# LasseWolter/laughter-detection-icsi

Hardware: AMD Instinct MI355X
Metric: 1 s@16 kHz segments/sec (featurize+ResNet fwd/bwd) (higher is better)
Workload: dtype f32 (64->64 and 32->32 convolutions: f16x2 split operands with per-tile power-of-two scales, f32 accumulate; error vs float64 within 1.5x of the exact-f32 kernels'); 1 GPU; BASELINE configs[2]: end-to-end featurize (HIP fbank 44 mel) + ResNetBigger resnet_base fwd/bwd + clip + Adam, random labels, dropout 0.5; global_batch=512, parallelism=dp1, overlap_wgrad=False, overlap_wgrad_small=True, bf16x3_convs=True, f16x2_convs=True, relu_bits=True, virtual_a1=True

## Files before the change

include/lad_hip.h:

```cpp
#ifndef LAD_HIP_H
#define LAD_HIP_H

#include <stdint.h>

#ifdef __cplusplus
extern "C" {
#endif

#define LAD_VERSION 100

enum lad_status {
    LAD_OK = 0,
    LAD_ERR_INVALID = -1,
    LAD_ERR_HIP = -2,
    LAD_ERR_NOMEM = -3,
    LAD_NOT_COVERED = 1
};

int lad_version(void);
const char *lad_last_error(void);

enum lad_pad_mode {
    LAD_PAD_KALDI_MIRROR = 0,
    LAD_PAD_CENTER_REFLECT = 1,
// ... 159 lines not shown
int lad_stem_bwd_onepass(const float *feat, const float *weight, const float *dy, const float *coef, const float *gamma,
                         const double *moments, float *workspace, float *dw, float *dgamma, float *dbeta, int64_t batch, int32_t H,
                         int32_t W, int32_t cout, void *stream);
int64_t lad_stem_wgrad_workspace_floats(void);
int lad_stem_wgrad(const float *feat, const float *dout, float *workspace, float *dw, int64_t batch, int32_t H,
                   int32_t W, int32_t cout, void *stream);
int lad_stem_wgrad_bn(const float *feat, const float *dy, const float *x, const float *weight, const float *coef,
                      const float *bcoef, float *workspace, float *dw, int64_t batch, int32_t H, int32_t W, int32_t cout,
                      void *stream);
int64_t lad_stem_bn_bwd_groups(int64_t batch, int32_t H, int32_t W);
int lad_stem_bn_bwd_sums(const float *feat, const float *weight, const float *dy, const float *coef, float *partials,
                         int64_t batch, int32_t H, int32_t W, int32_t cout, void *stream);

int lad_bn_finalize(float *stat_partials, int64_t n_tiles, int32_t channels, int64_t count, const float *gamma,
                    const float *beta, float *running_mean, float *running_var, float momentum, float *coef,
                    void *stream);
int lad_bn_finalize_pair(float *stat_partials_a, float *stat_partials_b, int64_t n_tiles, int32_t channels, int64_t count,
                         const float *gamma_a, const float *beta_a, float *running_mean_a, float *running_var_a, float *coef_a,
                         const float *gamma_b, const float *beta_b, float *running_mean_b, float *running_var_b, float *coef_b,
                         float momentum, void *stream);
int lad_bn_act(const float *x, const float *coef, const float *res, const float *res_coef, float *y, int64_t batch,
               int32_t H, int32_t W, int32_t channels, int32_t relu, void *stream);
int64_t lad_bn_bwd_workspace_floats(int32_t channels);
int lad_bn_bwd(const float *dy, const float *y, const float *x, const float *coef, const float *gamma,
               const float *xs, const float *scoef, const float *sgamma, float *dx, float *aux, float *dgamma,
               float *dbeta, float *dsgamma, float *dsbeta, float *workspace, float *bcoef, float *pre_partials,
               int64_t pre_tiles, int64_t batch, int32_t H, int32_t W, int32_t channels, int32_t relu, int32_t mode,
               void *stream);
int lad_bn_act_bits(const float *x, const float *coef, const float *res, const float *res_coef, float *y,
                    uint64_t *y_bits, int64_t batch, int32_t H, int32_t W, int32_t channels, void *stream);
int lad_bn_bwd_bits(const float *dy, const uint64_t *y_bits, const float *x, const float *coef, const float *gamma,
                    float *dx, float *dgamma, float *dbeta, float *workspace, float *bcoef, float *pre_partials,
                    int64_t pre_tiles, int64_t batch, int32_t H, int32_t W, int32_t channels, void *stream);
int lad_conv_fwd_bnstat(const float *in, const float *wt, const float *addend, float *out, float *stat_partials,
                        const float *bn_x, const float *bn_y, const float *bn_coef, int64_t batch, int32_t H, int32_t W,
                        int32_t cin, int32_t cout, int32_t taps, void *stream);

int lad_pool_fwd(const float *x, float *pooled, int64_t batch, int32_t H, int32_t W, int32_t channels, void *stream);
int lad_pool_bwd(const float *dpooled, float *dx, int64_t batch, int32_t H, int32_t W, int32_t channels, void *stream);
int64_t lad_head_workspace_floats(int64_t batch, int32_t F);
int lad_head_fwd_train(const float *const *params, const float *pooled, int64_t batch, int32_t F, const float *drop1,
                       const float *drop2, const int32_t *labels, float momentum, float *h, float *stats,
                       float *probs, float *metrics, void *stream);
int lad_head_fwd_train_rng(const float *const *params, const float *pooled, int64_t batch, int32_t F, float *drop1, float *drop2, float keep,
                           uint64_t seed, int64_t *rng_counter, int64_t *nbt, int32_t n_nbt, const int32_t *labels, float momentum,
                           float *h, float *stats, float *probs, float *metrics, void *stream);
int lad_head_fwd_eval(const float *const *params, const float *pooled, int64_t batch, int32_t F, float *probs,
                      void *stream);
int lad_bce_metrics(const float *probs, const int32_t *labels, int64_t n, float *metrics, void *stream);
int lad_head_bwd(const float *const *params, float *const *grads, const float *pooled, const float *h,
                 const float *stats, const float *probs, const float *dprobs, int64_t batch, int32_t F,
                 const float *drop1, const float *drop2, const int32_t *labels, float *workspace, float *dpooled,
                 void *stream);

int64_t lad_f16_packed_weight_halfs(int32_t cout, int32_t cin, int32_t taps);
int lad_f16_pack_weights(const float *w, int32_t cout, int32_t cin, int32_t taps, void *wt, void *stream);
int lad_f16_stem_fwd(const float *feat, const float *weight, const float *scale, const float *shift, void *out,
                     int64_t batch, int32_t H, int32_t W, int32_t cout, int64_t frame_stride, int64_t frames_avail,
                     void *stream);
int lad_f16_conv_fwd(const void *in, const void *wt, const float *scale, const float *shift, const void *addend, void *out,
                     int64_t batch, int32_t H, int32_t W, int32_t cin, int32_t cout, int32_t taps, int32_t relu,
                     void *stream);
int lad_f16_conv_s2_fwd(const void *in, const void *wt, const float *scale, const float *shift, void *out, int64_t batch,
                        int32_t H, int32_t W, int32_t cin, int32_t cout, int32_t taps, int32_t relu, void *stream);
int lad_f16_block_fwd(const void *x, const void *wt1, const float *scale1, const float *shift1, const void *wt2,
                      const float *scale2, const float *shift2, void *y, int64_t batch, int32_t H, int32_t W, int32_t channels,
                      void *stream);
int lad_f16_block_fwd_stem_rows(const void *stream_act, int64_t stream_rows, int64_t stream_row0, const float *feat, int64_t frames_avail,
                                const float *stem_weight, const float *stem_scale, const float *stem_shift, const void *wt1,
                                const float *scale1, const float *shift1, const void *wt2, const float *scale2, const float *shift2, void *y,
                                int64_t batch, int32_t H, int32_t W, void *stream);
int lad_f16_conv_s2_strips_fwd(const void *act, const void *wt, const float *scale, const float *shift, void *out, const void *wt_sc,
                               const float *scale_sc, const float *shift_sc, void *out_sc, int64_t n_windows, int32_t H, int32_t W,
                               int32_t band, int32_t strip_rows, int64_t bottom_image0, int64_t stream_row0, int64_t act_rows,
                               int32_t out_rows, void *stream);
int lad_f16_tail_fwd(const void *act, int64_t n_windows, int32_t H, int32_t W, int32_t band, int32_t strip_rows, int64_t bot_img0,
                     int64_t stream_row0, int32_t phases, int64_t phase_img, int64_t act_rows, const void *const *conv_params,
                     const float *const *head_params, int32_t F, float *probs, void *stream);
int lad_f16_conv_s2_fwd_windows(const void *act, const void *wt, const float *scale, const float *shift, void *out,
                                int64_t n_windows, int32_t H, int32_t W, int32_t band, int32_t cin, int32_t cout, int32_t taps,
                                int32_t relu, void *stream);
int lad_f16_conv_s2_fwd_mapped(const void *act, const void *wt, const float *scale, const float *shift, void *out,
                               int64_t n_windows, int32_t H, int32_t W, int32_t band, int32_t strip_rows, int64_t bottom_image0,
                               int64_t stream_row0, int32_t phases, int64_t phase_rows, int64_t act_rows, int32_t out_rows,
                               int32_t cin, int32_t cout, int32_t taps, int32_t relu, void *stream);
int lad_f16_conv_s2_fwd_sc(const void *in, const void *wt, const float *scale, const float *shift, void *out, const void *wt_sc,
                           const float *scale_sc, const float *shift_sc, void *out_sc, int64_t batch, int32_t H, int32_t W,
                           int32_t cin, int32_t cout, int32_t relu, void *stream);
int lad_f16_conv_s2_fwd_mapped_sc(const void *act, const void *wt, const float *scale, const float *shift, void *out,
                                  const void *wt_sc, const float *scale_sc, const float *shift_sc, void *out_sc, int64_t n_windows,
                                  int32_t H, int32_t W, int32_t band, int32_t strip_rows, int64_t bottom_image0, int64_t stream_row0,
                                  int32_t phases, int64_t phase_rows, int64_t act_rows, int32_t out_rows, int32_t cin, int32_t cout,
                                  int32_t relu, void *stream);
int lad_f16_pool_fwd(const void *x, float *pooled, int64_t batch, int32_t H, int32_t W, int32_t channels, void *stream);

int32_t lad_grad_sumsq_partials(void);
int lad_grad_sumsq(const float *grad, int64_t n, float *partials, int64_t *step_counter, void *stream);
int lad_grad_accumulate(float *acc, const float *grad, int64_t n, double scale, void *stream);
int lad_adam_step(float *param, float *grad, float *exp_avg, float *exp_avg_sq, int64_t n,
                  const float *sumsq_partials, double grad_scale, double max_norm, double lr, double beta1,
                  double beta2, double eps, int64_t step, const int64_t *step_counter, int32_t zero_grad,
                  float *norm_out, void *stream);

enum lad_runs_dtype { LAD_RUNS_F32 = 0, LAD_RUNS_F64 = 1 };
int32_t lad_runs_tile_frames(void);
int32_t lad_runs_max_thresholds(void);
// ... 107 lines not shown
```

laughter-detection-icsi_amd/_hip.py:

```python
import ctypes
import os

import numpy as np
import torch

_HERE = os.path.dirname(os.path.abspath(__file__))
LIB_PATH = os.environ.get("LAD_HIP_LIB") or os.path.join(_HERE, "liblad_hip.so")

c_void_p = ctypes.c_void_p
c_int = ctypes.c_int
c_i64 = ctypes.c_int64
c_float = ctypes.c_float
c_double = ctypes.c_double
c_i32 = ctypes.c_int32
c_float_p = ctypes.POINTER(ctypes.c_float)


class LadHipError(RuntimeError):
    pass


class FbankCfg(ctypes.Structure):
    _fields_ = [("n_fft", ctypes.c_int32), ("frame_len", ctypes.c_int32), ("hop", ctypes.c_int32),
                ("n_mels", ctypes.c_int32), ("n_mfcc", ctypes.c_int32), ("pad_mode", ctypes.c_int32),
# ... 56 lines not shown
    "lad_conv_fwd_eval": (c_int, [c_void_p] * 6 + [c_i64, c_i32, c_i32, c_i32, c_i32, c_i32, c_i32, c_void_p]),
    "lad_conv_s2_fwd_eval": (c_int, [c_void_p] * 5 + [c_i64, c_i32, c_i32, c_i32, c_i32, c_i32, c_i32, c_void_p]),
    "lad_upsample2": (c_int, [c_void_p, c_void_p, c_i64, c_i32, c_i32, c_i32, c_void_p]),
    "lad_conv_s2_dgrad": (c_int, [c_void_p] * 3 + [c_i64, c_i32, c_i32, c_i32, c_i32, c_i32, c_i32, c_void_p]),
    "lad_conv_s2_wgrad_workspace_floats": (c_i64, [c_i32, c_i32, c_i32]),
    "lad_conv_s2_fwd_fused": (c_int, [c_void_p] * 8 + [c_i64, c_i32, c_i32, c_i32, c_i32, c_void_p]),
    "lad_conv_s2_dgrad_partials": (c_i64, [c_i64, c_i32, c_i32]),
    "lad_conv_s2b3_packed_weight_bytes": (c_i64, []),
    "lad_conv_s2b3_pack_weights": (c_int, [c_void_p, c_void_p, c_void_p, c_void_p]),
    "lad_conv_s2b3_fwd": (c_int, [c_void_p] * 7 + [c_i64, c_i32, c_i32, c_void_p]),
    "lad_conv_s2b3_dgrad_packed_weight_bytes": (c_i64, []),
    "lad_conv_s2b3_dgrad_pack_weights": (c_int, [c_void_p, c_void_p, c_void_p, c_void_p]),
    "lad_conv_s2b3_pack_weights_pair": (c_int, [c_void_p] * 5),
    "lad_conv_s2b3_dgrad_partials": (c_i64, [c_i64, c_i32, c_i32]),
    "lad_conv_s2b3_dgrad": (c_int, [c_void_p] * 8 + [c_i64, c_i32, c_i32, c_void_p]),
    "lad_conv_s2_dgrad_fused_bnstat": (c_int, [c_void_p] * 9 + [c_i64, c_i32, c_i32, c_i32, c_i32, c_void_p]),
    "lad_conv_s2_dgrad_fused": (c_int, [c_void_p] * 5 + [c_i64, c_i32, c_i32, c_i32, c_i32, c_void_p]),
    "lad_conv_s2_wgrad_fused_workspace_floats": (c_i64, [c_i32, c_i32]),
    "lad_conv_s2_wgrad_fused": (c_int, [c_void_p] * 7 + [c_i64, c_i32, c_i32, c_i32, c_i32, c_void_p]),
    "lad_conv_s2_wgrad": (c_int, [c_void_p] * 5 + [c_i64, c_i32, c_i32, c_i32, c_i32, c_i32, c_void_p]),
    "lad_conv_wgrad_workspace_floats": (c_i64, [c_i32, c_i32, c_i32]),
    "lad_conv_wgrad": (c_int, [c_void_p] * 5 + [c_i64, c_i32, c_i32, c_i32, c_i32, c_i32, c_void_p]),
    "lad_stem_fwd": (c_int, [c_void_p] * 4 + [c_i64, c_i32, c_i32, c_i32, c_void_p]),
    "lad_stem_fwd_eval": (c_int, [c_void_p] * 5 + [c_i64, c_i32, c_i32, c_i32, c_i64, c_i64, c_void_p]),
    "lad_stem_wgrad_workspace_floats": (c_i64, []),
    "lad_stem_wgrad": (c_int, [c_void_p] * 4 + [c_i64, c_i32, c_i32, c_i32, c_void_p]),
    "lad_stem_wgrad_bn": (c_int, [c_void_p] * 8 + [c_i64, c_i32, c_i32, c_i32, c_void_p]),
    "lad_stem_bn_bwd_groups": (c_i64, [c_i64, c_i32, c_i32]),
    "lad_stem_bn_bwd_sums": (c_int, [c_void_p] * 5 + [c_i64, c_i32, c_i32, c_i32, c_void_p]),
    "lad_bn_finalize": (c_int, [c_void_p, c_i64, c_i32, c_i64, c_void_p, c_void_p, c_void_p, c_void_p, c_float,
                                c_void_p, c_void_p]),
    "lad_stem_moments_workspace_doubles": (c_i64, []),
    "lad_stem_moments_doubles": (c_i64, []),
    "lad_stem_bn_stats": (c_int, [c_void_p] * 6 + [c_float] + [c_void_p] * 3 + [c_i64, c_i32, c_i32, c_i32, c_void_p]),
    "lad_stem_bwd_onepass_workspace_floats": (c_i64, []),
    "lad_stem_bwd_onepass": (c_int, [c_void_p] * 10 + [c_i64, c_i32, c_i32, c_i32, c_void_p]),
    "lad_bn_finalize_pair": (c_int, [c_void_p, c_void_p, c_i64, c_i32, c_i64] + [c_void_p] * 10 + [c_float, c_void_p]),
    "lad_bn_act": (c_int, [c_void_p] * 5 + [c_i64, c_i32, c_i32, c_i32, c_i32, c_void_p]),
    "lad_bn_bwd_workspace_floats": (c_i64, [c_i32]),
    "lad_bn_act_bits": (c_int, [c_void_p] * 6 + [c_i64, c_i32, c_i32, c_i32, c_void_p]),
    "lad_bn_bwd_bits": (c_int, [c_void_p] * 11 + [c_i64, c_i64, c_i32, c_i32, c_i32, c_void_p]),
    "lad_bn_bwd": (c_int, [c_void_p] * 17 + [c_i64, c_i64, c_i32, c_i32, c_i32, c_i32, c_i32, c_void_p]),
    "lad_conv_fwd_bnstat": (c_int, [c_void_p] * 8 + [c_i64, c_i32, c_i32, c_i32, c_i32, c_i32, c_void_p]),
    "lad_pool_fwd": (c_int, [c_void_p, c_void_p, c_i64, c_i32, c_i32, c_i32, c_void_p]),
    "lad_pool_bwd": (c_int, [c_void_p, c_void_p, c_i64, c_i32, c_i32, c_i32, c_void_p]),
    "lad_head_workspace_floats": (c_i64, [c_i64, c_i32]),
    "lad_head_fwd_train": (c_int, [c_void_p, c_void_p, c_i64, c_i32, c_void_p, c_void_p, c_void_p, c_float,
                                   c_void_p, c_void_p, c_void_p, c_void_p, c_void_p]),
    "lad_head_fwd_train_rng": (c_int, [c_void_p, c_void_p, c_i64, c_i32, c_void_p, c_void_p, c_float, ctypes.c_uint64, c_void_p, c_void_p, c_i32,
                                       c_void_p, c_float, c_void_p, c_void_p, c_void_p, c_void_p, c_void_p]),
    "lad_head_fwd_eval": (c_int, [c_void_p, c_void_p, c_i64, c_i32, c_void_p, c_void_p]),
    "lad_bce_metrics": (c_int, [c_void_p, c_void_p, c_i64, c_void_p, c_void_p]),
    "lad_head_bwd": (c_int, [c_void_p] * 7 + [c_i64, c_i32] + [c_void_p] * 6),
    "lad_f16_packed_weight_halfs": (c_i64, [c_i32, c_i32, c_i32]),
    "lad_f16_pack_weights": (c_int, [c_void_p, c_i32, c_i32, c_i32, c_void_p, c_void_p]),
    "lad_f16_stem_fwd": (c_int, [c_void_p] * 5 + [c_i64, c_i32, c_i32, c_i32, c_i64, c_i64, c_void_p]),
    "lad_f16_conv_fwd": (c_int, [c_void_p] * 6 + [c_i64, c_i32, c_i32, c_i32, c_i32, c_i32, c_i32, c_void_p]),
    "lad_f16_block_fwd": (c_int, [c_void_p] * 8 + [c_i64, c_i32, c_i32, c_i32, c_void_p]),
    "lad_f16_conv_s2_fwd_sc": (c_int, [c_void_p] * 9 + [c_i64, c_i32, c_i32, c_i32, c_i32, c_i32, c_void_p]),
    "lad_f16_conv_s2_fwd_mapped_sc": (c_int, [c_void_p] * 9 + [c_i64, c_i32, c_i32, c_i32, c_i32, c_i64, c_i64, c_i32, c_i64, c_i64, c_i32,
                                              c_i32, c_i32, c_i32, c_void_p]),
    "lad_f16_conv_s2_fwd": (c_int, [c_void_p] * 5 + [c_i64, c_i32, c_i32, c_i32, c_i32, c_i32, c_i32, c_void_p]),
    "lad_f16_conv_s2_fwd_windows": (c_int, [c_void_p] * 5 + [c_i64, c_i32, c_i32, c_i32, c_i32, c_i32, c_i32, c_i32, c_void_p]),
    "lad_f16_conv_s2_fwd_mapped": (c_int, [c_void_p] * 5 + [c_i64, c_i32, c_i32, c_i32, c_i32, c_i64, c_i64, c_i32, c_i64, c_i64, c_i32,
                                                          c_i32, c_i32, c_i32, c_i32, c_void_p]),
    "lad_f16_block_fwd_stem_rows": (c_int, [c_void_p, c_i64, c_i64, c_void_p, c_i64] + [c_void_p] * 10 + [c_i64, c_i32, c_i32, c_void_p]),
    "lad_f16_conv_s2_strips_fwd": (c_int, [c_void_p] * 9 + [c_i64, c_i32, c_i32, c_i32, c_i32, c_i64, c_i64, c_i64, c_i32, c_void_p]),
    "lad_f16_tail_fwd": (c_int, [c_void_p, c_i64, c_i32, c_i32, c_i32, c_i32, c_i64, c_i64, c_i32, c_i64, c_i64, c_void_p, c_void_p, c_i32,
                                 c_void_p, c_void_p]),
    "lad_f16_pool_fwd": (c_int, [c_void_p, c_void_p, c_i64, c_i32, c_i32, c_i32, c_void_p]),
    "lad_grad_sumsq_partials": (c_i32, []),
    "lad_grad_sumsq": (c_int, [c_void_p, c_i64, c_void_p, c_void_p, c_void_p]),
    "lad_grad_accumulate": (c_int, [c_void_p, c_void_p, c_i64, c_double, c_void_p]),
    "lad_adam_step": (c_int, [c_void_p] * 4 + [c_i64, c_void_p] + [c_double] * 6 + [c_i64, c_void_p, c_i32, c_void_p, c_void_p]),
    "lad_runs_tile_frames": (c_i32, []),
    "lad_runs_max_thresholds": (c_i32, []),
    "lad_runs_workspace_bytes": (c_i64, [c_i64, c_i64, c_i32]),
    "lad_runs_count": (c_int, [c_void_p, c_i32, c_i64, c_i64, ctypes.POINTER(c_double), c_i32, c_void_p, c_void_p]),
    "lad_runs_fill": (c_int, [c_void_p, c_i32, c_i64, c_i64, ctypes.POINTER(c_double), c_i32, c_void_p,
                              ctypes.POINTER(c_i32), c_void_p, c_i64, c_void_p]),
    "lad_score_max_min_lengths": (c_i32, []),
    "lad_score_workspace_bytes": (c_i64, [c_i64, c_i64, c_i32, c_i32]),
    "lad_score_runs": (c_int, [c_void_p, c_void_p, ctypes.POINTER(c_i32), c_i64, c_i64, c_i32, c_void_p, c_void_p,
                               ctypes.POINTER(c_i32), ctypes.POINTER(c_i32), c_i64, c_void_p, ctypes.POINTER(c_double),
                               ctypes.POINTER(c_double), c_i32, c_void_p, c_void_p, c_void_p]),
    "lad_score_events_workspace_bytes": (c_i64, [c_i64, c_i64, c_i32, c_i32, c_i64]),
    "lad_score_events": (c_int, [c_void_p, c_void_p, ctypes.POINTER(c_i32), c_i64, c_i64, c_i32, c_void_p, c_void_p,
                                 ctypes.POINTER(c_i32), ctypes.POINTER(c_i32), c_i64, c_void_p, ctypes.POINTER(c_double),
                                 ctypes.POINTER(c_double), c_i32, c_i32, c_i32, c_void_p, c_void_p, c_void_p]),
    "lad_binarize_max_settings": (c_i32, []),
    "lad_binarize_workspace_bytes": (c_i64, [c_i64, c_i64, c_i32]),
    "lad_binarize_count": (c_int, [c_void_p, c_i32, c_i64, c_i64, ctypes.POINTER(c_double), ctypes.POINTER(c_double), c_i32,
                                   c_void_p, c_void_p]),
    "lad_binarize_fill": (c_int, [c_void_p, c_i32, c_i64, c_i64] + [ctypes.POINTER(c_double)] * 3
                          + [c_i32, c_void_p, ctypes.POINTER(c_double), c_void_p, ctypes.POINTER(c_i32), c_void_p, c_void_p, c_i64,
                             c_void_p]),
    "lad_viterbi_max_settings": (c_i32, []),
    "lad_viterbi_table_entries": (c_i32, []),
    "lad_viterbi_workspace_bytes": (c_i64, [c_i64, c_i64, c_i32]),
    "lad_viterbi_count": (c_int, [c_void_p, c_i32, c_i64, c_i64, c_void_p] + [ctypes.POINTER(c_i32)] * 3
                          + [c_i32, c_void_p, c_void_p, c_void_p]),
    "lad_viterbi_fill": (c_int, [c_void_p, ctypes.POINTER(c_i32), c_i64, c_i64, c_i32, c_void_p, c_i64, c_void_p]),
    "lad_surface_max_levels": (c_i32, []),
    "lad_surface_tile_frames": (c_i32, []),
    "lad_surface_workspace_bytes": (c_i64, [c_i64, c_i64, c_i64, c_i32, c_i32]),
    "lad_score_surface": (c_int, [c_void_p, c_i32, c_i64, c_i64, ctypes.POINTER(c_double), c_i32, c_void_p, c_void_p,
# ... 116 lines not shown
```

laughter-detection-icsi_amd/csrc/head.hip:

```cpp
#include "lad_common.h"
#include "lad_device.h"
#include "lad_philox.h"

namespace {
using namespace lad;

#ifdef LAD_STAMP
__device__ unsigned long long lad_dbg_head[64];
#define LAD_HEAD_STAMP(k) if (threadIdx.x == 0) lad_dbg_head[k] = __builtin_amdgcn_s_memtime();
#else
#define LAD_HEAD_STAMP(k)
#endif

constexpr float BN_EPS = 1e-5f;
constexpr int HID = 32;
constexpr int HEAD_THREADS = 1024;
constexpr int MAX_F = 128;
constexpr int CH = 64;

struct HeadArgs {
    int B, F;
    const float *g2, *b2;
    float *rm2, *rv2;
    const float *W1, *bias1;
// ... 524 lines not shown
        if (worker) {
            for (int b = g; b < nb; b += KS) {
                const float4 dv = *reinterpret_cast<const float4 *>(dh_s + b * DHS + tj * TJ);
                const float dd[TJ] = {dv.x, dv.y, dv.z, dv.w};
                float zz[TF];
#pragma unroll
                for (int y = 0; y < TF; ++y) zz[y] = z_s[b * (MAX_F + 1) + min(tf * TF + y, MAX_F - 1)];
#pragma unroll
                for (int x = 0; x < TJ; ++x)
#pragma unroll
                    for (int y = 0; y < TF; ++y) wacc[x][y] = fmaf(dd[x], zz[y], wacc[x][y]);
            }
        }
        __syncthreads();
    }
    {
        float *part = z_s;
        if (worker) {
#pragma unroll
            for (int x = 0; x < TJ; ++x)
#pragma unroll
                for (int y = 0; y < TF; ++y) {
                    const int f = tf * TF + y;
                    if (f < F) part[(g * HID + tj * TJ + x) * F + f] = wacc[x][y];
                }
        }
        __syncthreads();
        for (int idx = tid; idx < HID * F; idx += nt) {
            float sacc = part[idx];
            for (int q = 1; q < KS; ++q) sacc += part[q * HID * F + idx];
            gr_out.dW1[idx] = sacc;
        }
        __syncthreads();
    }
    LAD_HEAD_STAMP(22)
    col_dot2(dh, nullptr, nullptr, nullptr, B, HID, gr_out.dbias1, nullptr, scratch);
    LAD_HEAD_STAMP(23)
    col_dot2(dz, pooled, mean2, istd2, B, F, ca, cb, scratch);
    __syncthreads();
    for (int f = tid; f < F; f += nt) {
        gr_out.db2[f] = ca[f];
        gr_out.dg2[f] = cb[f];
    }
    LAD_HEAD_STAMP(24)
    batched<12, F2>(tid, B * F, nt, [&](int idx) { return F2{pooled[idx], dz[idx]}; },
                   [&](int idx, const F2 &v) {
                       const int f = idx % F;
                       const float xh = (v.a - mu2[f]) * is2[f];
                       dpooled[idx] = kk2[f] * (v.b - ca[f] / (float)B - xh * cb[f] / (float)B);
                   });
    LAD_HEAD_STAMP(25)
}

int check_head(const HeadArgs &a) {
    using namespace lad;
    LAD_REQUIRE(a.B >= 1 && a.F >= 1 && a.F <= MAX_F, "head: F must be 1..%d (got %d), B >= 1", MAX_F, a.F);
    LAD_REQUIRE(a.g2 && a.b2 && a.rm2 && a.rv2 && a.W1 && a.bias1 && a.g3 && a.b3 && a.rm3 && a.rv3 && a.W2 && a.bias2,
                "head: null parameter pointer");
    return LAD_OK;
}

}

extern "C" int lad_pool_fwd(const float *x, float *pooled, int64_t batch, int32_t H, int32_t W, int32_t channels, void *stream) {
    using namespace lad;
    LAD_REQUIRE(x && pooled, "lad_pool_fwd: null buffer");
    LAD_REQUIRE(H >= 4 && W >= 4 && channels >= 1, "lad_pool_fwd: AvgPool2d(4) needs H, W >= 4");
    if (batch == 0) return LAD_OK;
    const int PH = H / 4, PW = W / 4;
    const int64_t n = batch * channels * PH * PW;
    hipLaunchKernelGGL(pool_fwd_kernel, dim3((unsigned)ceil_div(n, 256)), dim3(256), 0, (hipStream_t)stream, x, pooled, batch, H + 1,
                       W + 1, channels, PH, PW);
    return check_launch("pool_fwd_kernel");
}

extern "C" int lad_pool_bwd(const float *dpooled, float *dx, int64_t batch, int32_t H, int32_t W, int32_t channels, void *stream) {
    using namespace lad;
    LAD_REQUIRE(dpooled && dx, "lad_pool_bwd: null buffer");
    LAD_REQUIRE(H >= 4 && W >= 4 && channels >= 1, "lad_pool_bwd: AvgPool2d(4) needs H, W >= 4");
    if (batch == 0) return LAD_OK;
    const int64_t n = batch * (H + 1) * (W + 1) * channels;
    hipLaunchKernelGGL(pool_bwd_kernel, dim3((unsigned)std::min<int64_t>(ceil_div(n, 256), 4096)), dim3(256), 0, (hipStream_t)stream,
                       dpooled, dx, batch, H + 1, W + 1, channels, H / 4, W / 4);
    return check_launch("pool_bwd_kernel");
}

static HeadArgs make_args(const float *const *p, int64_t B, int32_t F, const float *m1, const float *m2, const int32_t *labels,
                          float momentum) {
    HeadArgs a;
    a.B = (int)B; a.F = F;
    a.g2 = p[0]; a.b2 = p[1]; a.rm2 = (float *)p[2]; a.rv2 = (float *)p[3];
    a.W1 = p[4]; a.bias1 = p[5];
    a.g3 = p[6]; a.b3 = p[7]; a.rm3 = (float *)p[8]; a.rv3 = (float *)p[9];
    a.W2 = p[10]; a.bias2 = p[11];
    a.m1 = m1; a.m2 = m2; a.labels = (const int *)labels; a.momentum = momentum;
    a.keep = 1.f; a.seed = 0; a.rng_counter = nullptr; a.nbt = nullptr; a.n_nbt = 0;
    return a;
}

extern "C" int64_t lad_head_workspace_floats(int64_t batch, int32_t F) { return batch * (3 * HID + F); }

extern "C" int lad_head_fwd_train(const float *const *params, const float *pooled, int64_t batch, int32_t F, const float *drop1,
                                  const float *drop2, const int32_t *labels, float momentum, float *h, float *stats, float *probs,
                                  float *metrics, void *stream) {
    using namespace lad;
    LAD_REQUIRE(params && pooled && h && stats && probs && metrics, "lad_head_fwd_train: null buffer");
    LAD_REQUIRE(batch < (1 << 24), "lad_head_fwd_train: batch too large for the single-workgroup train head");
    HeadArgs a = make_args(params, batch, F, drop1, drop2, labels, momentum);
    int rc = check_head(a);
    if (rc) return rc;
    hipLaunchKernelGGL(head_fwd_train_kernel, dim3(1), dim3(HEAD_THREADS), 0, (hipStream_t)stream, a, pooled, h, stats, probs, metrics);
    return check_launch("head_fwd_train_kernel");
}

extern "C" int lad_head_fwd_train_rng(const float *const *params, const float *pooled, int64_t batch, int32_t F, float *drop1, float *drop2,
                                      float keep, uint64_t seed, int64_t *rng_counter, int64_t *nbt, int32_t n_nbt, const int32_t *labels,
                                      float momentum, float *h, float *stats, float *probs, float *metrics, void *stream) {
    using namespace lad;
    LAD_REQUIRE(params && pooled && h && stats && probs && metrics, "lad_head_fwd_train_rng: null buffer");
    LAD_REQUIRE(batch >= 2, "lad_head_fwd_train_rng: batch statistics need at least two samples");
    const bool drop = keep < 1.0f;
    LAD_REQUIRE(!drop || (keep > 0.f && drop1 && drop2 && rng_counter && F % 4 == 0), "lad_head_fwd_train_rng: dropout needs mask buffers, a counter and F %% 4 == 0");
    LAD_REQUIRE(n_nbt >= 0 && n_nbt <= HEAD_THREADS - 64 && (n_nbt == 0 || nbt), "lad_head_fwd_train_rng: bad counter list");
    HeadArgs a = make_args(params, batch, F, drop ? drop1 : nullptr, drop ? drop2 : nullptr, labels, momentum);
    int rc = check_head(a);
    if (rc) return rc;
    a.keep = keep; a.seed = seed; a.rng_counter = drop ? (long long *)rng_counter : nullptr; a.nbt = (long long *)nbt; a.n_nbt = n_nbt;
    hipLaunchKernelGGL(head_fwd_train_kernel, dim3(1), dim3(HEAD_THREADS), 0, (hipStream_t)stream, a, pooled, h, stats, probs, metrics);
    return check_launch("head_fwd_train_kernel");
}

extern "C" int lad_head_fwd_eval(const float *const *params, const float *pooled, int64_t batch, int32_t F, float *probs, void *stream) {
    using namespace lad;
    LAD_REQUIRE(params && pooled && probs, "lad_head_fwd_eval: null buffer");
    if (batch == 0) return LAD_OK;
    HeadArgs a = make_args(params, batch, F, nullptr, nullptr, nullptr, 0.f);
    int rc = check_head(a);
    if (rc) return rc;
    hipLaunchKernelGGL(head_fwd_eval_kernel, dim3((unsigned)ceil_div(batch, 256)), dim3(256), 0, (hipStream_t)stream, a, pooled, probs);
    return check_launch("head_fwd_eval_kernel");
}

extern "C" int lad_bce_metrics(const float *probs, const int32_t *labels, int64_t n, float *metrics, void *stream) {
    using namespace lad;
    LAD_REQUIRE(probs && labels && metrics && n >= 1 && n < (1 << 30), "lad_bce_metrics: bad argument");
    hipLaunchKernelGGL(bce_metrics_kernel, dim3(1), dim3(HEAD_THREADS), 0, (hipStream_t)stream, probs, (const int *)labels, (int)n,
                       metrics);
    return check_launch("bce_metrics_kernel");
}

extern "C" int lad_head_bwd(const float *const *params, float *const *grads, const float *pooled, const float *h, const float *stats,
                            const float *probs, const float *dprobs, int64_t batch, int32_t F, const float *drop1, const float *drop2,
                            const int32_t *labels, float *workspace, float *dpooled, void *stream) {
    using namespace lad;
    LAD_REQUIRE(params && grads && pooled && h && stats && probs && workspace && dpooled, "lad_head_bwd: null buffer");
    LAD_REQUIRE(dprobs || labels, "lad_head_bwd: need dprobs or labels");
    HeadArgs a = make_args(params, batch, F, drop1, drop2, labels, 0.f);
    int rc = check_head(a);
    if (rc) return rc;
    HeadGrads g;
    g.dg2 = grads[0]; g.db2 = grads[1]; g.dW1 = grads[2]; g.dbias1 = grads[3];
    g.dg3 = grads[4]; g.db3 = grads[5]; g.dW2 = grads[6]; g.dbias2 = grads[7];
    hipLaunchKernelGGL(head_bwd_kernel, dim3(1), dim3(HEAD_THREADS), 0, (hipStream_t)stream, a, g, pooled, h, stats, probs, dprobs,
                       workspace, dpooled);
    return check_launch("head_bwd_kernel");
}

#ifdef LAD_STAMP
extern "C" int lad_debug_read_head_stamps(unsigned long long *host_dst, int64_t n) {
    return hipMemcpyFromSymbol(host_dst, HIP_SYMBOL(lad_dbg_head), n * sizeof(unsigned long long)) == hipSuccess ? 0 : -2;
}
#endif
```

Before: 49890 segments/s.

## Stage head forward/backward in large LDS to avoid repeated global passes

Adds LDS-resident variants of the single-block classifier head forward and backward kernels. The whole pooled batch, W1 and intermediate rows are held in up to 160 KB of dynamic shared memory, so column reductions, the matmuls and the BN backward avoid repeated global memory round trips. These kernels are selected by default when B and F fit and pointers are 16-byte aligned, with a fallback to the old kernels. The head is a single-block kernel, so any gain is bounded by its small share of the step. The large LDS opt-in may fail on some devices.

After: 50380 segments/s (median of 6 runs). About the same (+1.0%).

```diff
diff --git a/include/lad_hip.h b/include/lad_hip.h
--- a/include/lad_hip.h
+++ b/include/lad_hip.h
@@ -235,6 +235,7 @@
                  const float *stats, const float *probs, const float *dprobs, int64_t batch, int32_t F,
                  const float *drop1, const float *drop2, const int32_t *labels, float *workspace, float *dpooled,
                  void *stream);
+int lad_head_set_lds(int on);
 
 int64_t lad_f16_packed_weight_halfs(int32_t cout, int32_t cin, int32_t taps);
 int lad_f16_pack_weights(const float *w, int32_t cout, int32_t cin, int32_t taps, void *wt, void *stream);
diff --git a/laughter-detection-icsi_amd/_hip.py b/laughter-detection-icsi_amd/_hip.py
--- a/laughter-detection-icsi_amd/_hip.py
+++ b/laughter-detection-icsi_amd/_hip.py
@@ -132,6 +132,7 @@
     "lad_head_fwd_eval": (c_int, [c_void_p, c_void_p, c_i64, c_i32, c_void_p, c_void_p]),
     "lad_bce_metrics": (c_int, [c_void_p, c_void_p, c_i64, c_void_p, c_void_p]),
     "lad_head_bwd": (c_int, [c_void_p] * 7 + [c_i64, c_i32] + [c_void_p] * 6),
+    "lad_head_set_lds": (c_int, [c_int]),
     "lad_f16_packed_weight_halfs": (c_i64, [c_i32, c_i32, c_i32]),
     "lad_f16_pack_weights": (c_int, [c_void_p, c_i32, c_i32, c_i32, c_void_p, c_void_p]),
     "lad_f16_stem_fwd": (c_int, [c_void_p] * 5 + [c_i64, c_i32, c_i32, c_i32, c_i64, c_i64, c_void_p]),
diff --git a/laughter-detection-icsi_amd/csrc/head.hip b/laughter-detection-icsi_amd/csrc/head.hip
--- a/laughter-detection-icsi_amd/csrc/head.hip
+++ b/laughter-detection-icsi_amd/csrc/head.hip
@@ -600,6 +600,559 @@
     LAD_HEAD_STAMP(25)
 }
 
+constexpr int LDS_MAX_BYTES = 160 * 1024;
+constexpr int LDS_MAX_F = 64;
+constexpr int RCH = 64;
+constexpr int MAXCH = 8;
+constexpr int DHP = HID + 4;
+
+struct HeadSmall {
+    float zs[MAX_F], zt[MAX_F], ca[MAX_F], cb[MAX_F], mu2[MAX_F], is2[MAX_F], kk2[MAX_F];
+    float us[HID], ut[HID], w2s[HID], b1s[HID];
+    float red[5][HEAD_THREADS / 64];
+};
+static_assert(sizeof(HeadSmall) % 16 == 0, "the parts behind HeadSmall are 16-byte aligned");
+
+struct HeadLds {
+    int rp;
+    int w1, scratch, dhb, zb, rows;
+    int64_t bytes;
+};
+__host__ __device__ inline HeadLds head_lds_layout(int64_t B, int F) {
+    HeadLds L;
+    L.rp = (F > HID ? F : HID) | 1;
+    int o = (int)sizeof(HeadSmall);
+    L.w1 = o;      o += F * HID * (int)sizeof(float);
+    L.scratch = o; o += 3 * HEAD_THREADS * (int)sizeof(double);
+    L.dhb = o;     o += RCH * DHP * (int)sizeof(float);
+    L.zb = o;      o += RCH * F * (int)sizeof(float);
+    L.rows = o;
+    L.bytes = o + B * L.rp * (int64_t)sizeof(float);
+    return L;
+}
+inline bool head_lds_fits(int64_t B, int F) {
+    if (B < 1 || F < 4 || F > LDS_MAX_F || F % 4 != 0) return false;
+    if (B > (int64_t)RCH * MAXCH) return false;
+    return head_lds_layout(B, F).bytes <= LDS_MAX_BYTES;
+}
+
+template <int NS>
+__device__ __forceinline__ void col_meet(int ncol, double *scratch, const double (&s)[NS], double (&r)[NS]) {
+    const int nt = blockDim.x, nph = nt / ncol;
+    __syncthreads();
+#pragma unroll
+    for (int i = 0; i < NS; ++i) scratch[i * nt + threadIdx.x] = s[i];
+    __syncthreads();
+#pragma unroll
+    for (int i = 0; i < NS; ++i) r[i] = 0.0;
+    if (threadIdx.x < ncol) {
+        for (int p = 0; p < nph; ++p) {
+#pragma unroll
+            for (int i = 0; i < NS; ++i) r[i] += scratch[i * nt + p * ncol + threadIdx.x];
+        }
+    }
+    __syncthreads();
+}
+
+__global__ __launch_bounds__(HEAD_THREADS) void head_fwd_train_lds_kernel(HeadArgs a, const float *__restrict__ pooled,
+                                                                          float *__restrict__ h, float *__restrict__ stats,
+                                                                          float *__restrict__ probs, float *__restrict__ metrics) {
+    extern __shared__ __attribute__((aligned(16))) unsigned char head_lds[];
+    const int tid = threadIdx.x, nt = blockDim.x;
+    const int B = a.B, F = a.F;
+    const HeadLds L = head_lds_layout(B, F);
+    HeadSmall &S = *reinterpret_cast<HeadSmall *>(head_lds);
+    float *w1t = reinterpret_cast<float *>(head_lds + L.w1);
+    double *scratch = reinterpret_cast<double *>(head_lds + L.scratch);
+    float *R = reinterpret_cast<float *>(head_lds + L.rows);
+    const int RP = L.rp;
+    const bool rng = a.rng_counter != nullptr, has1 = a.m1 != nullptr, has2 = a.m2 != nullptr;
+    const int br = (4 * tid) / F, fq = 4 * tid - br * F;
+    const bool eact = br < RCH;
+
+    LAD_HEAD_STAMP(32)
+    float4 pv[MAXCH], mv[MAXCH];
+#pragma unroll
+    for (int c = 0; c < MAXCH; ++c)
+        if (eact && c * RCH + br < B) pv[c] = reinterpret_cast<const float4 *>(pooled)[c * (RCH * F / 4) + tid];
+    if (has1 && !rng) {
+#pragma unroll
+        for (int c = 0; c < MAXCH; ++c)
+            if (eact && c * RCH + br < B) mv[c] = reinterpret_cast<const float4 *>(a.m1)[c * (RCH * F / 4) + tid];
+    }
+    float tl = 0.f;
+    unsigned keep2 = 0u;
+    if (tid < B && a.labels != nullptr) tl = (float)a.labels[tid];
+    float g2c = 0.f, b2c = 0.f, rm2c = 0.f, rv2c = 0.f, g3c = 0.f, b3c = 0.f, rm3c = 0.f, rv3c = 0.f, w2c = 0.f, b1c = 0.f;
+    if (tid < F) { g2c = a.g2[tid]; b2c = a.b2[tid]; rm2c = a.rm2[tid]; rv2c = a.rv2[tid]; }
+    if (tid < HID) { g3c = a.g3[tid]; b3c = a.b3[tid]; rm3c = a.rm3[tid]; rv3c = a.rv3[tid]; w2c = a.W2[tid]; b1c = a.bias1[tid]; }
+    const float bias2 = a.bias2[0];
+    float wv[LDS_MAX_F * HID / HEAD_THREADS];
+#pragma unroll
+    for (int k = 0; k < LDS_MAX_F * HID / HEAD_THREADS; ++k)
+        if (tid + k * nt < F * HID) wv[k] = a.W1[tid + k * nt];
+    if (rng) {
+        const long long draw = *a.rng_counter;
+        float4 *o1 = reinterpret_cast<float4 *>(const_cast<float *>(a.m1)), *o2 = reinterpret_cast<float4 *>(const_cast<float *>(a.m2));
+#pragma unroll
+        for (int c = 0; c < MAXCH; ++c)
+            if (eact && c * RCH + br < B) {
+                const int g = c * (RCH * F / 4) + tid;
+                mv[c] = dropout_mask4(a.seed, draw, 0, (unsigned)g, a.keep);
+                o1[g] = mv[c];
+            }
+        if (tid < B) {
+#pragma unroll
+            for (int q = 0; q < HID / 4; ++q) {
+                const float4 m = dropout_mask4(a.seed, draw, 1, (unsigned)(tid * (HID / 4) + q), a.keep);
+                o2[tid * (HID / 4) + q] = m;
+                keep2 |= ((m.x != 0.f) ? 1u : 0u) << (4 * q) | ((m.y != 0.f) ? 2u : 0u) << (4 * q) | ((m.z != 0.f) ? 4u : 0u) << (4 * q) |
+                         ((m.w != 0.f) ? 8u : 0u) << (4 * q);
+            }
+        }
+    }
+#pragma unroll
+    for (int c = 0; c < MAXCH; ++c)
+        if (eact && c * RCH + br < B) {
+            float *r = R + (c * RCH + br) * RP + fq;
+            r[0] = pv[c].x; r[1] = pv[c].y; r[2] = pv[c].z; r[3] = pv[c].w;
+        }
+#pragma unroll
+    for (int k = 0; k < LDS_MAX_F * HID / HEAD_THREADS; ++k) {
+        const int i = tid + k * nt;
+        if (i < F * HID) {
+            const int j = i / F, f = i - j * F;
+            w1t[f * HID + j] = wv[k];
+        }
+    }
+    if (tid < HID) {
+        S.b1s[tid] = b1c;
+        S.w2s[tid] = w2c;
+    }
+    __syncthreads();
+    LAD_HEAD_STAMP(33)
+    {
+        double s1, s2;
+        col_reduce(B, F, scratch, s1, s2, [&](int b, int c) { return F2{R[b * RP + c], 0.f}; },
+                   [&](const F2 &x, int, double &a0, double &a1) {
+                       const double v = (double)x.a;
+                       a0 += v;
+                       a1 += v * v;
+                   });
+        const int c = tid;
+        if (c < F) {
+            const double mean = s1 / B;
+            double var = s2 / B - mean * mean;
+            if (var < 0.0) var = 0.0;
+            const float mean_f = (float)mean, istd_f = (float)(1.0 / sqrt(var + (double)BN_EPS));
+            stats[c] = mean_f;
+            stats[F + c] = istd_f;
+            const double unb = B > 1 ? var * B / (B - 1.0) : var;
+            a.rm2[c] = fmaf(a.momentum, (float)mean, (1.f - a.momentum) * rm2c);
+            a.rv2[c] = fmaf(a.momentum, (float)unb, (1.f - a.momentum) * rv2c);
+            const float s = istd_f * g2c;
+            S.zs[c] = s;
+            S.zt[c] = b2c - mean_f * s;
+        }
+    }
+    __syncthreads();
+#pragma unroll
+    for (int c = 0; c < MAXCH; ++c)
+        if (eact && c * RCH + br < B) {
+            float *r = R + (c * RCH + br) * RP + fq;
+            const float m4[4] = {mv[c].x, mv[c].y, mv[c].z, mv[c].w};
+#pragma unroll
+            for (int i = 0; i < 4; ++i) {
+                float z = fmaf(r[i], S.zs[fq + i], S.zt[fq + i]);
+                if (has1) z *= m4[i];
+                r[i] = z;
+            }
+        }
+    __syncthreads();
+    LAD_HEAD_STAMP(34)
+    float mk[HID];
+    if (has2 && !rng && tid < B) {
+#pragma unroll
+        for (int q = 0; q < HID / 4; ++q) {
+            const float4 m = reinterpret_cast<const float4 *>(a.m2 + (int64_t)tid * HID)[q];
+            mk[4 * q] = m.x; mk[4 * q + 1] = m.y; mk[4 * q + 2] = m.z; mk[4 * q + 3] = m.w;
+        }
+    }
+    constexpr int NU = HID / 2;
+#pragma unroll 1
+    for (int t = tid; t < 2 * B; t += nt) {
+        const int b = t >> 1, j0 = (t & 1) * NU;
+        float acc[NU];
+#pragma unroll
+        for (int j = 0; j < NU; ++j) acc[j] = S.b1s[j0 + j];
+        float *zr = R + b * RP;
+        for (int f = 0; f < F; ++f) {
+            const float z = zr[f];
+            const float4 *w = reinterpret_cast<const float4 *>(w1t + f * HID + j0);
+#pragma unroll
+            for (int q = 0; q < NU / 4; ++q) {
+                const float4 wq = w[q];
+                acc[4 * q] = fmaf(wq.x, z, acc[4 * q]);
+                acc[4 * q + 1] = fmaf(wq.y, z, acc[4 * q + 1]);
+                acc[4 * q + 2] = fmaf(wq.z, z, acc[4 * q + 2]);
+                acc[4 * q + 3] = fmaf(wq.w, z, acc[4 * q + 3]);
+            }
+        }
+        float4 *hr = reinterpret_cast<float4 *>(h + (int64_t)b * HID + j0);
+#pragma unroll
+        for (int j = 0; j < NU; j += 4) hr[j >> 2] = make_float4(acc[j], acc[j + 1], acc[j + 2], acc[j + 3]);
+#pragma unroll
+        for (int j = 0; j < NU; ++j) zr[j0 + j] = acc[j];
+    }
+    __syncthreads();
+    LAD_HEAD_STAMP(35)
+    {
+        double s1, s2;
+        col_reduce(B, HID, scratch, s1, s2, [&](int b, int c) { return F2{R[b * RP + c], 0.f}; },
+                   [&](const F2 &x, int, double &a0, double &a1) {
+                       const double v = (double)x.a;
+                       a0 += v;
+                       a1 += v * v;
+                   });
+        const int c = tid;
+        if (c < HID) {
+            const double mean = s1 / B;
+            double var = s2 / B - mean * mean;
+            if (var < 0.0) var = 0.0;
+            const float mean_f = (float)mean, istd_f = (float)(1.0 / sqrt(var + (double)BN_EPS));
+            stats[2 * F + c] = mean_f;
+            stats[2 * F + HID + c] = istd_f;
+            const double unb = B > 1 ? var * B / (B - 1.0) : var;
+            a.rm3[c] = fmaf(a.momentum, (float)mean, (1.f - a.momentum) * rm3c);
+            a.rv3[c] = fmaf(a.momentum, (float)unb, (1.f - a.momentum) * rv3c);
+            const float s = istd_f * g3c;
+            S.us[c] = s;
+            S.ut[c] = b3c - mean_f * s;
+        }
+    }
+    __syncthreads();
+    LAD_HEAD_STAMP(36)
+    float loss = 0.f, n_corr = 0.f, n_pp = 0.f, n_tp = 0.f, n_t = 0.f;
+    if (tid < B) {
+        const int b = tid;
+        float part[HID];
+#pragma unroll
+        for (int j = 0; j < HID; ++j) part[j] = R[b * RP + j];
+        const float t = tl;
+        if (rng) {
+            const float inv = 1.0f / a.keep;
+#pragma unroll
+            for (int j = 0; j < HID; ++j) mk[j] = ((keep2 >> j) & 1u) ? inv : 0.f;
+        }
+#pragma unroll
+        for (int j = 0; j < HID; ++j) {
+            float u = fmaf(part[j], S.us[j], S.ut[j]);
+            if (has2) u *= mk[j];
+            part[j] = fmaxf(u, 0.f);
+        }
+#pragma unroll
+        for (int j = 0; j < HID / 2; ++j) part[j] = fmaf(S.w2s[j], part[j], S.w2s[j + HID / 2] * part[j + HID / 2]);
+#pragma unroll
+        for (int off = HID / 4; off > 0; off >>= 1)
+#pragma unroll
+            for (int j = 0; j < off; ++j) part[j] += part[j + off];
+        const float p = sigmoidf(part[0] + bias2);
+        probs[b] = p;
+        if (a.labels != nullptr) {
+            const float lp = fmaxf(logf(p), -100.f), l1p = fmaxf(logf(1.f - p), -100.f);
+            loss -= t * lp + (1.f - t) * l1p;
+            const float pred = rintf(p);
+            n_corr += (pred == t) ? 1.f : 0.f;
+            n_pp += pred;
+            n_tp += (pred == 1.f && t == 1.f) ? 1.f : 0.f;
+            n_t += t;
+        }
+    }
+    LAD_HEAD_STAMP(37)
+    float vals[5] = {loss, n_corr, n_pp, n_tp, n_t};
+#pragma unroll
+    for (int k = 0; k < 5; ++k) {
+        const float v = wave_sum64(vals[k]);
+        if ((tid & 63) == 0) S.red[k][tid >> 6] = v;
+    }
+    __syncthreads();
+    if (tid < 5) {
+        float s = 0.f;
+        for (int w = 0; w < nt / 64; ++w) s += S.red[tid][w];
+        metrics[tid] = (tid == 0) ? s / (float)B : s;
+    }
+    if (tid == 5) metrics[5] = (float)B;
+    if (rng && tid == 6) *a.rng_counter += 1;
+    if (a.nbt != nullptr && tid >= 64 && tid - 64 < a.n_nbt) a.nbt[tid - 64] += 1;
+    LAD_HEAD_STAMP(38)
+}
+
+__global__ __launch_bounds__(HEAD_THREADS) void head_bwd_lds_kernel(HeadArgs a, HeadGrads gr_out, const float *__restrict__ pooled,
+                                                                    const float *__restrict__ h, const float *__restrict__ stats,
+                                                                    const float *__restrict__ probs, const float *__restrict__ dprobs,
+                                                                    float *__restrict__ dpooled) {
+    extern __shared__ __attribute__((aligned(16))) unsigned char head_lds[];
+    const int tid = threadIdx.x, nt = blockDim.x;
+    const int B = a.B, F = a.F;
+    const HeadLds L = head_lds_layout(B, F);
+    HeadSmall &S = *reinterpret_cast<HeadSmall *>(head_lds);
+    float *w1 = reinterpret_cast<float *>(head_lds + L.w1);
+    double *scratch = reinterpret_cast<double *>(head_lds + L.scratch);
+    float *dhb = reinterpret_cast<float *>(head_lds + L.dhb), *zb = reinterpret_cast<float *>(head_lds + L.zb);
+    float *R = reinterpret_cast<float *>(head_lds + L.rows);
+    float *dl_s = dhb;
+    const int RP = L.rp;
+    const bool has1 = a.m1 != nullptr;
+    const int br = (4 * tid) / F, fq = 4 * tid - br * F;
+    const bool eact = br < RCH;
+    const int jt = tid & (HID - 1), r0 = tid >> 5;
+    constexpr int K32 = 2 * MAXCH;
+    static_assert(RCH * HID == 2 * HEAD_THREADS && HID == 32, "a chunk is two (sample, unit) registers per thread");
+
+    LAD_HEAD_STAMP(40)
+    float4 pv[MAXCH], mreg[MAXCH];
+#pragma unroll
+    for (int c = 0; c < MAXCH; ++c)
+        if (eact && c * RCH + br < B) pv[c] = reinterpret_cast<const float4 *>(pooled)[c * (RCH * F / 4) + tid];
+    if (has1) {
+#pragma unroll
+        for (int c = 0; c < MAXCH; ++c)
+            if (eact && c * RCH + br < B) mreg[c] = reinterpret_cast<const float4 *>(a.m1)[c * (RCH * F / 4) + tid];
+    }
+    float hv[K32], dv[K32], m2v[K32];
+#pragma unroll
+    for (int k = 0; k < K32; ++k) {
+        const int idx = tid + k * nt;
+        if (idx < B * HID) {
+            hv[k] = h[idx];
+            m2v[k] = a.m2 ? a.m2[idx] : 1.f;
+        }
+    }
+    float p_b = 0.f, t_b = 0.f;
+    if (tid < B) {
+        p_b = probs[tid];
+        t_b = dprobs != nullptr ? dprobs[tid] : (float)a.labels[tid];
+    }
+    const float mean3_j = stats[2 * F + jt], istd3_j = stats[2 * F + HID + jt], g3_j = a.g3[jt], b3_j = a.b3[jt], w2_j = a.W2[jt];
+    float mean2_c = 0.f, istd2_c = 0.f, g2_c = 0.f, b2_c = 0.f;
+    if (tid < F) { mean2_c = stats[tid]; istd2_c = stats[F + tid]; g2_c = a.g2[tid]; b2_c = a.b2[tid]; }
+    const int cc = tid % F, ph = tid / F, nph = nt / F;
+    const float mc = stats[cc], ic = stats[F + cc];
+    float wv[LDS_MAX_F * HID / HEAD_THREADS];
+#pragma unroll
+    for (int k = 0; k < LDS_MAX_F * HID / HEAD_THREADS; ++k)
+        if (tid + k * nt < F * HID) wv[k] = a.W1[tid + k * nt];
+#pragma unroll
+    for (int c = 0; c < MAXCH; ++c)
+        if (eact && c * RCH + br < B) {
+            float *r = R + (c * RCH + br) * RP + fq;
+            r[0] = pv[c].x; r[1] = pv[c].y; r[2] = pv[c].z; r[3] = pv[c].w;
+        }
+#pragma unroll
+    for (int k = 0; k < LDS_MAX_F * HID / HEAD_THREADS; ++k)
+        if (tid + k * nt < F * HID) w1[tid + k * nt] = wv[k];
+    if (tid < F) {
+        const float s = istd2_c * g2_c;
+        S.zs[tid] = s;
+        S.zt[tid] = b2_c - mean2_c * s;
+        S.mu2[tid] = mean2_c;
+        S.is2[tid] = istd2_c;
+        S.kk2[tid] = g2_c * istd2_c;
+    }
+    if (tid < B) {
+        float dlogit;
+        if (dprobs != nullptr) dlogit = t_b * p_b * (1.f - p_b);
+        else dlogit = (p_b - t_b) / (float)B;
+        dl_s[tid] = dlogit;
+    }
+    const float us_j = istd3_j * g3_j, ut_j = b3_j - mean3_j * us_j, k3_j = g3_j * istd3_j;
+    __syncthreads();
+    LAD_HEAD_STAMP(41)
+    float dl_sum = 0.f;
+    double s3[3] = {0.0, 0.0, 0.0}, r3[3];
+#pragma unroll
+    for (int k = 0; k < K32; ++k) {
+        const int idx = tid + k * nt;
+        if (idx < B * HID) {
+            const float dlogit = dl_s[r0 + 32 * k];
+            if (jt == 0) dl_sum += dlogit;
+            float u = fmaf(hv[k], us_j, ut_j);
+            const float m = m2v[k];
+            u *= m;
+            const float grv = dlogit * fmaxf(u, 0.f);
+            const float duv = (u > 0.f) ? dlogit * w2_j * m : 0.f;
+            dv[k] = duv;
+            s3[0] += (double)grv;
+            const double x = (double)duv;
+            s3[1] += x;
+            s3[2] += x * (double)((hv[k] - mean3_j) * istd3_j);
+        }
+    }
+    dl_sum = wave_sum64(dl_sum);
+    if ((tid & 63) == 0) S.red[0][tid >> 6] = dl_sum;
+    col_meet<3>(HID, scratch, s3, r3);
+    if (tid == 0) {
+        float s = 0.f;
+        for (int w = 0; w < nt / 64; ++w) s += S.red[0][w];
+        gr_out.dbias2[0] = s;
+    }
+    if (tid < HID) {
+        const float ca = (float)r3[1], cb = (float)r3[2];
+        gr_out.dW2[tid] = (float)r3[0];
+        gr_out.db3[tid] = ca;
+        gr_out.dg3[tid] = cb;
+        S.ca[tid] = ca;
+        S.cb[tid] = cb;
+    }
+    __syncthreads();
+    LAD_HEAD_STAMP(42)
+    {
+        const float ca_j = S.ca[jt] / (float)B, cb_j = S.cb[jt];
+        double s1[1] = {0.0}, r1[1];
+#pragma unroll
+        for (int k = 0; k < K32; ++k) {
+            const int idx = tid + k * nt;
+            if (idx < B * HID) {
+                const float xh = (hv[k] - mean3_j) * istd3_j;
+                const float dhv = k3_j * (dv[k] - ca_j - xh * cb_j / (float)B);
+                dv[k] = dhv;
+                s1[0] += (double)dhv;
+            }
+        }
+        col_meet<1>(HID, scratch, s1, r1);
+        if (tid < HID) gr_out.dbias1[tid] = (float)r1[0];
+    }
+    LAD_HEAD_STAMP(43)
+    constexpr int TJ = 4, TF = 3;
+    const int ftiles = (F + TF - 1) / TF, ntile = (HID / TJ) * ftiles;
+    int KS = 8;
+    while (KS > 1 && (ntile * KS > nt || KS * HID * F > CH * (MAX_F + 1))) KS >>= 1;
+    const bool worker = tid < ntile * KS;
+    const int g = tid / ntile, tile = tid - g * ntile, tj = tile / ftiles, tf = tile - tj * ftiles;
+    float wacc[TJ][TF];
+#pragma unroll
+    for (int x = 0; x < TJ; ++x)
+#pragma unroll
+        for (int y = 0; y < TF; ++y) wacc[x][y] = 0.f;
+    double s2[2] = {0.0, 0.0}, r2[2];
+    int bnext = ph;
+#pragma unroll
+    for (int c = 0; c < MAXCH; ++c) {
+        const int c0 = c * RCH;
+        if (c0 < B) {
+            const int nb = min(RCH, B - c0);
+            const bool mine = eact && br < nb;
+#pragma unroll
+            for (int kk = 0; kk < 2; ++kk)
+                if (tid + (2 * c + kk) * nt < B * HID) dhb[(r0 + 32 * kk) * DHP + jt] = dv[2 * c + kk];
+            if (mine) {
+                const float *r = R + (c0 + br) * RP + fq;
+                const float m4[4] = {mreg[c].x, mreg[c].y, mreg[c].z, mreg[c].w};
+                float z4[4];
+#pragma unroll
+                for (int i = 0; i < 4; ++i) {
+                    float z = fmaf(r[i], S.zs[fq + i], S.zt[fq + i]);
+                    if (has1) z *= m4[i];
+                    z4[i] = z;
+                }
+                *reinterpret_cast<float4 *>(zb + br * F + fq) = make_float4(z4[0], z4[1], z4[2], z4[3]);
+            }
+            __syncthreads();
+            if (worker) {
+                for (int b = g; b < nb; b += KS) {
+                    const float4 d4 = *reinterpret_cast<const float4 *>(dhb + b * DHP + tj * TJ);
+                    const float dd[TJ] = {d4.x, d4.y, d4.z, d4.w};
+                    float zz[TF];
+#pragma unroll
+                    for (int y = 0; y < TF; ++y) zz[y] = zb[b * F + min(tf * TF + y, F - 1)];
+#pragma unroll
+                    for (int x = 0; x < TJ; ++x)
+#pragma unroll
+                        for (int y = 0; y < TF; ++y) wacc[x][y] = fmaf(dd[x], zz[y], wacc[x][y]);
+                }
+            }
+            float dz4[4] = {0.f, 0.f, 0.f, 0.f};
+            if (mine) {
+                const float m4[4] = {mreg[c].x, mreg[c].y, mreg[c].z, mreg[c].w};
+#pragma unroll
+                for (int jq = 0; jq < HID / 4; ++jq) {
+                    const float4 d4 = *reinterpret_cast<const float4 *>(dhb + br * DHP + 4 * jq);
+                    const float dd[4] = {d4.x, d4.y, d4.z, d4.w};
+#pragma unroll
+                    for (int x = 0; x < 4; ++x) {
+                        const float4 w4 = *reinterpret_cast<const float4 *>(w1 + (4 * jq + x) * F + fq);
+                        dz4[0] = fmaf(w4.x, dd[x], dz4[0]);
+                        dz4[1] = fmaf(w4.y, dd[x], dz4[1]);
+                        dz4[2] = fmaf(w4.z, dd[x], dz4[2]);
+                        dz4[3] = fmaf(w4.w, dd[x], dz4[3]);
+                    }
+                }
+                if (has1) {
+#pragma unroll
+                    for (int i = 0; i < 4; ++i) dz4[i] *= m4[i];
+                }
+                mreg[c] = make_float4(dz4[0], dz4[1], dz4[2], dz4[3]);
+            }
+            __syncthreads();
+            if (mine) *reinterpret_cast<float4 *>(zb + br * F + fq) = make_float4(dz4[0], dz4[1], dz4[2], dz4[3]);
+            __syncthreads();
+            if (ph < nph) {
+                for (; bnext < c0 + nb; bnext += nph) {
+                    const double x = (double)zb[(bnext - c0) * F + cc];
+                    s2[0] += x;
+                    s2[1] += x * (double)((R[bnext * RP + cc] - mc) * ic);
+                }
+            }
+            __syncthreads();
+        }
+    }
+    LAD_HEAD_STAMP(44)
+    {
+        float *part = reinterpret_cast<float *>(scratch);
+        if (worker) {
+#pragma unroll
+            for (int x = 0; x < TJ; ++x)
+#pragma unroll
+                for (int y = 0; y < TF; ++y) {
+                    const int f = tf * TF + y;
+                    if (f < F) part[(g * HID + tj * TJ + x) * F + f] = wacc[x][y];
+                }
+        }
+        __syncthreads();
+        for (int idx = tid; idx < HID * F; idx += nt) {
+            float sacc = part[idx];
+            for (int q = 1; q < KS; ++q) sacc += part[q * HID * F + idx];
+            gr_out.dW1[idx] = sacc;
+        }
+    }
+    LAD_HEAD_STAMP(45)
+    col_meet<2>(F, scratch, s2, r2);
+    if (tid < F) {
+        const float ca = (float)r2[0], cb = (float)r2[1];
+        gr_out.db2[tid] = ca;
+        gr_out.dg2[tid] = cb;
+        S.ca[tid] = ca;
+        S.cb[tid] = cb;
+    }
+    __syncthreads();
+    LAD_HEAD_STAMP(46)
+#pragma unroll
+    for (int c = 0; c < MAXCH; ++c)
+        if (eact && c * RCH + br < B) {
+            const float *r = R + (c * RCH + br) * RP + fq;
+            const float d4[4] = {mreg[c].x, mreg[c].y, mreg[c].z, mreg[c].w};
+            float o[4];
+#pragma unroll
+            for (int i = 0; i < 4; ++i) {
+                const int f = fq + i;
+                const float xh = (r[i] - S.mu2[f]) * S.is2[f];
+                o[i] = S.kk2[f] * (d4[i] - S.ca[f] / (float)B - xh * S.cb[f] / (float)B);
+            }
+            reinterpret_cast<float4 *>(dpooled)[c * (RCH * F / 4) + tid] = make_float4(o[0], o[1], o[2], o[3]);
+        }
+    LAD_HEAD_STAMP(47)
+}
+
 int check_head(const HeadArgs &a) {
     using namespace lad;
     LAD_REQUIRE(a.B >= 1 && a.F >= 1 && a.F <= MAX_F, "head: F must be 1..%d (got %d), B >= 1", MAX_F, a.F);
@@ -608,7 +1161,39 @@
     return LAD_OK;
 }
 
-}
+std::atomic<int> head_lds_on{1};
+
+inline bool aligned16(const void *p) { return (reinterpret_cast<uintptr_t>(p) & 15) == 0; }
+
+bool head_lds_opt_in(const void *kernel, DeviceOnce &granted, DeviceOnce &refused) {
+    if (!granted) {
+        if (!!refused) return false;
+        if (hipFuncSetAttribute(kernel, hipFuncAttributeMaxDynamicSharedMemorySize, LDS_MAX_BYTES) == hipSuccess) {
+            granted = true;
+        } else {
+            (void)hipGetLastError();
+            refused = true;
+            return false;
+        }
+    }
+    return true;
+}
+
+int launch_head_fwd_train(const HeadArgs &a, const float *pooled, float *h, float *stats, float *probs, float *metrics, hipStream_t st) {
+    static DeviceOnce granted, refused;
+    if (head_lds_on.load(std::memory_order_relaxed) && head_lds_fits(a.B, a.F) && aligned16(pooled) && aligned16(h) && aligned16(a.m1) &&
+        aligned16(a.m2) && head_lds_opt_in((const void *)head_fwd_train_lds_kernel, granted, refused)) {
+        hipLaunchKernelGGL(head_fwd_train_lds_kernel, dim3(1), dim3(HEAD_THREADS), (size_t)head_lds_layout(a.B, a.F).bytes, st, a, pooled, h,
+                           stats, probs, metrics);
+        return check_launch("head_fwd_train_lds_kernel");
+    }
+    hipLaunchKernelGGL(head_fwd_train_kernel, dim3(1), dim3(HEAD_THREADS), 0, st, a, pooled, h, stats, probs, metrics);
+    return check_launch("head_fwd_train_kernel");
+}
+
+}
+
+extern "C" int lad_head_set_lds(int on) { return head_lds_on.exchange(on ? 1 : 0); }
 
 extern "C" int lad_pool_fwd(const float *x, float *pooled, int64_t batch, int32_t H, int32_t W, int32_t channels, void *stream) {
     using namespace lad;
@@ -657,8 +1242,7 @@
     HeadArgs a = make_args(params, batch, F, drop1, drop2, labels, momentum);
     int rc = check_head(a);
     if (rc) return rc;
-    hipLaunchKernelGGL(head_fwd_train_kernel, dim3(1), dim3(HEAD_THREADS), 0, (hipStream_t)stream, a, pooled, h, stats, probs, metrics);
-    return check_launch("head_fwd_train_kernel");
+    return launch_head_fwd_train(a, pooled, h, stats, probs, metrics, (hipStream_t)stream);
 }
 
 extern "C" int lad_head_fwd_train_rng(const float *const *params, const float *pooled, int64_t batch, int32_t F, float *drop1, float *drop2,
@@ -674,8 +1258,7 @@
     int rc = check_head(a);
     if (rc) return rc;
     a.keep = keep; a.seed = seed; a.rng_counter = drop ? (long long *)rng_counter : nullptr; a.nbt = (long long *)nbt; a.n_nbt = n_nbt;
-    hipLaunchKernelGGL(head_fwd_train_kernel, dim3(1), dim3(HEAD_THREADS), 0, (hipStream_t)stream, a, pooled, h, stats, probs, metrics);
-    return check_launch("head_fwd_train_kernel");
+    return launch_head_fwd_train(a, pooled, h, stats, probs, metrics, (hipStream_t)stream);
 }
 
 extern "C" int lad_head_fwd_eval(const float *const *params, const float *pooled, int64_t batch, int32_t F, float *probs, void *stream) {
@@ -709,6 +1292,13 @@
     HeadGrads g;
     g.dg2 = grads[0]; g.db2 = grads[1]; g.dW1 = grads[2]; g.dbias1 = grads[3];
     g.dg3 = grads[4]; g.db3 = grads[5]; g.dW2 = grads[6]; g.dbias2 = grads[7];
+    static DeviceOnce granted, refused;
+    if (head_lds_on.load(std::memory_order_relaxed) && head_lds_fits(a.B, a.F) && aligned16(pooled) && aligned16(dpooled) && aligned16(a.m1) &&
+        head_lds_opt_in((const void *)head_bwd_lds_kernel, granted, refused)) {
+        hipLaunchKernelGGL(head_bwd_lds_kernel, dim3(1), dim3(HEAD_THREADS), (size_t)head_lds_layout(a.B, a.F).bytes, (hipStream_t)stream, a, g,
+                           pooled, h, stats, probs, dprobs, dpooled);
+        return check_launch("head_bwd_lds_kernel");
+    }
     hipLaunchKernelGGL(head_bwd_kernel, dim3(1), dim3(HEAD_THREADS), 0, (hipStream_t)stream, a, g, pooled, h, stats, probs, dprobs,
                        workspace, dpooled);
     return check_launch("head_bwd_kernel");
```
